# idthanm/mpg

Hardware: AMD Instinct MI355X
Metric: env-steps/sec + grad-steps/sec, PathTrackingEnv MPG n=25 batch=4096 (higher is better)
Workload: dtype f32-via-split-f16; 1 GPU; PathTrackingEnv, MPG-v2 learner, n=25, M=1, 4096 vectorised envs + replay batch 4096 per GPU; step = worker.sample(4096 env-steps) + add_batch + replay + compute_gradient + (all-reduce) + apply_gradients; global_batch=4096, parallelism=dp1, grad_allreduce_floats=205334, native_step_driver=True, always_exchange=False, overlap_exchange=False, rows_per_gpu=4096

## Files before the change

### mpg_amd/csrc/fused_kernels.hip

```cpp
#include "mlp_wgrad.h"

namespace mlp {

namespace {

template <bool PK>
__device__ __forceinline__ void load_w2(const float* pack, const float* W2, bool bwd, const Lane& L, float (&w)[128]) {
    if constexpr (PK) load_w2_packed(pack, L, w);
    else if (bwd) load_w2_bwd(W2, L, w);
    else load_w2_fwd(W2, L, w);
}

#define MPG_UNPAREN(...) __VA_ARGS__
#define MPG_LOAD2(SMALL, IMAGE) do { MPG_UNPAREN SMALL; MPG_UNPAREN IMAGE; } while (0)


constexpr int SMEM_FLOATS = 2 * A_IMG + GROUP * XS + NWAVE * GROUP * MAXOUT + GROUP * MAXOUT + NWAVE * GROUP * XS + 4 * GROUP;
struct Smem {
    float *sA, *sA1, *sX, *sPart, *sD3, *sPartX, *sQ;
    __device__ explicit Smem(float* base) {
        sA = base;
        sA1 = sA + A_IMG;
        sX = sA1 + A_IMG;
        sPart = sX + GROUP * XS;
        sD3 = sPart + NWAVE * GROUP * MAXOUT;
        sPartX = sD3 + GROUP * MAXOUT;
        sQ = sPartX + NWAVE * GROUP * XS;
    }
};

struct TargetArgs {
    const float *pol, *q1, *q2;
    const float *pk_pol, *pk_q1, *pk_q2;
    int rows;
    const float *obs2, *rew, *smooth_eps;
    float scale[8];
    int out_tanh;
    float out_scale, sigma, clipc, rshift, rscale, gamma;
    float* y;
    int draw, n_storage;
    int d_capacity, d_fresh_start, d_fresh_count;
    uint32_t dk0, dk1, dc1, dc2;
    const float *r_obs, *r_act, *r_rew, *r_obs2;
    const uint8_t* r_done;
    int* o_idx;
    float *o_obs, *o_act, *o_rew, *o_obs2, *o_done;
    int* status;
    float* qpart;
    unsigned long long* dbg;
};

template <int OBS, int ACT, bool PK, int G2>
__global__ void __launch_bounds__(NTHREAD, 2) k_target_fused(const TargetArgs a) {
    constexpr int QIN = OBS + ACT;
    __shared__ __attribute__((aligned(16))) float smem[SMEM_FLOATS];
    __shared__ __attribute__((aligned(16))) float sXg[G2][GROUP * XS];
    __shared__ float sQg[G2][2 * GROUP];
    const Smem m(smem);
    const Lane L;
    const int tid = threadIdx.x;
    const long g0 = (long)blockIdx.x * G2;
    const int half = a.qpart ? (int)blockIdx.y : -1;
    __shared__ float sRew[G2 * GROUP];
    MPG_TL_DECL
    MPG_TL(0);
    float o1[OBS], o2[OBS], ac[ACT], rw = 0.f;
    uint8_t dn = 0;
    long sr = 0;
    bool saw_nan = false;
#pragma unroll
    for (int i = 0; i < OBS; ++i) o1[i] = o2[i] = 0.f;
#pragma unroll
    for (int k = 0; k < ACT; ++k) ac[k] = 0.f;
    const bool drawn = a.draw && tid < G2 * GROUP && g0 * GROUP + tid < a.rows;
    bool gather = drawn;
    if (drawn) {
        const long gr = g0 * GROUP + tid;
        const Philox4 p = philox4x32_10((uint32_t)(gr >> 2), a.dc1, a.dc2, 0x1d5u, a.dk0, a.dk1);
        sr = (long)(((uint64_t)philox_word(p, (int)(gr & 3)) * (uint64_t)a.n_storage) >> 32);
        if (a.draw == 2) {
            int off = (int)sr - a.d_fresh_start;
            if (off < 0) off += a.d_capacity;
            gather = off < a.d_fresh_count;
        }
        if (gather) {
#pragma unroll
            for (int i = 0; i < OBS; ++i) { o1[i] = a.r_obs[sr * OBS + i]; o2[i] = a.r_obs2[sr * OBS + i]; }
#pragma unroll
            for (int k = 0; k < ACT; ++k) ac[k] = a.r_act[sr * ACT + k];
            rw = a.r_rew[sr];
            dn = a.r_done[sr];
        } else {
#pragma unroll
            for (int i = 0; i < OBS; ++i) o2[i] = a.o_obs2[gr * OBS + i];
            rw = a.o_rew[gr];
        }
    }
    float w2[128], h1[2][4], h2[2][4];
    float zmax = 0.f;
    const Net pnet = make_net(a.pol, OBS, 2 * ACT);
    float pb3 = 0.f, qb3[2] = {0.f, 0.f}, sm_eps = 0.f;
    if (tid < G2 * GROUP * ACT) {
        pb3 = pnet.b3[tid % ACT];
        const long gr0 = (g0 + tid / (GROUP * ACT)) * GROUP + (tid / ACT) % GROUP;
        if (a.smooth_eps && gr0 < a.rows) sm_eps = a.smooth_eps[gr0 * ACT + tid % ACT];
    }
    if (tid < G2 * GROUP) {
        qb3[0] = make_net(a.q1, OBS + ACT, 1).b3[0];
        if (a.q2) qb3[1] = make_net(a.q2, OBS + ACT, 1).b3[0];
    }
    SmallRegs<OBS, ACT> pr;
    MPG_TL(1);
    MPG_LOAD2((load_small<OBS, ACT>(pnet, L, pr)), (load_w2<PK>(a.pk_pol, pnet.W2, false, L, w2)));
    MPG_TL(2);
    if (a.draw) {
        if (tid < G2 * GROUP) {
            if (gather && half <= 0) {
                const long gr = g0 * GROUP + tid;
                if (a.o_idx) a.o_idx[gr] = (int)sr;
#pragma unroll
                for (int i = 0; i < OBS; ++i) { a.o_obs[gr * OBS + i] = o1[i]; a.o_obs2[gr * OBS + i] = o2[i]; }
#pragma unroll
                for (int k = 0; k < ACT; ++k) a.o_act[gr * ACT + k] = ac[k];
                a.o_rew[gr] = rw;
                if (a.o_done) a.o_done[gr] = (float)dn;
            }
            sRew[tid] = rw;
            saw_nan |= rw != rw;
#pragma unroll
            for (int i = 0; i < XS; ++i) sXg[tid / GROUP][(tid % GROUP) * XS + i] = i < OBS ? o2[i < OBS ? i : 0] * a.scale[i] : 0.f;
#pragma unroll
            for (int i = 0; i < OBS; ++i) saw_nan |= o2[i] != o2[i];
        }
    } else if (tid < G2 * GROUP * XS) {
        const int g2 = tid / (GROUP * XS), e = tid % (GROUP * XS), row = e / XS, i = e % XS;
        const long gr = (g0 + g2) * GROUP + row;
        const float xin = (gr < a.rows && i < OBS) ? a.obs2[gr * OBS + i] * a.scale[i] : 0.f;
        sXg[g2][e] = xin;
        saw_nan |= xin != xin;
        if (i == 0) {
            const float rin = gr < a.rows ? a.rew[gr] : 0.f;
            sRew[g2 * GROUP + row] = rin;
            saw_nan |= rin != rin;
        }
    }
    MPG_TL(3);
    lds_barrier();
    MPG_TL(4);
    float h1b[2][4], h2b[2][4];
    if constexpr (G2 == 2) {
        forward_group2<OBS, ACT>(sXg[0], sXg[1], m.sA, m.sA1, m.sPart, m.sPartX, L, w2, pr, h1, h2, h1b, h2b, &zmax);
    } else {
        forward_group<OBS, ACT>(sXg[0], m.sA, m.sPart, L, w2, pr, h1, h2, nullptr, 0, nullptr, &zmax);
    }
    if (tid < G2 * GROUP * ACT) {
        const int g2 = tid / (GROUP * ACT), row = (tid / ACT) % GROUP, k = tid % ACT;
        const long gr = (g0 + g2) * GROUP + row;
        const float z = out_preact(g2 == 0 ? m.sPart : m.sPartX, pb3, row, k);
        float act = a.out_tanh ? a.out_scale * tanhf(z) : z;
        if (a.smooth_eps && gr < a.rows) act += fminf(fmaxf(a.sigma * sm_eps, -a.clipc), a.clipc);
        sXg[g2][row * XS + OBS + k] = act;
    }
    MPG_TL(5);
    lds_barrier();
    MPG_TL(6);
#pragma unroll
    for (int qi = 0; qi < 2; ++qi) {
        const float* qp = qi == 0 ? a.q1 : a.q2;
        if (!qp) break;
        if (half >= 0 && qi != half) continue;
        const Net net = make_net(qp, QIN, 1);
        SmallRegs<QIN, 1> r;
        MPG_LOAD2((load_small<QIN, 1>(net, L, r)), (load_w2<PK>(qi == 0 ? a.pk_q1 : a.pk_q2, net.W2, false, L, w2)));
        MPG_TL(10 + 6 * qi);
        if constexpr (G2 == 2) {
            forward_group2<QIN, 1>(sXg[0], sXg[1], m.sA, m.sA1, m.sPart, m.sPartX, L, w2, r, h1, h2, h1b, h2b, &zmax);
        } else {
            forward_group<QIN, 1>(sXg[0], m.sA, m.sPart, L, w2, r, h1, h2, nullptr, 0, nullptr, &zmax);
        }
        if (tid < G2 * GROUP) {
            const int g2 = tid / GROUP, row = tid % GROUP;
            sQg[g2][qi * GROUP + row] = out_preact(g2 == 0 ? m.sPart : m.sPartX, qb3[qi], row, 0);
        }
        MPG_TL(11 + 6 * qi);
        lds_barrier();
        MPG_TL(12 + 6 * qi);
    }
    MPG_TL(22);
    if (tid < G2 * GROUP) {
        const int g2 = tid / GROUP, row = tid % GROUP;
        const long gr = (g0 + g2) * GROUP + row;
        if (gr < a.rows) {
            const float pz = row_poison(sXg[g2] + row * XS, OBS);
            if (half >= 0) a.qpart[(long)half * a.rows + gr] = sQg[g2][half * GROUP + row] + pz;
            else {
                const float q = a.q2 ? fminf(sQg[g2][row], sQg[g2][GROUP + row]) : sQg[g2][row];
                a.y[gr] = (sRew[tid] + a.rshift) * a.rscale + a.gamma * q + pz;
            }
        }
    }
    report_activation_range(a.status, zmax);
    report_nan(a.status, saw_nan);
    MPG_TL(23);
    MPG_TL_DUMP(a.dbg);
}

struct QlossArgs {
    const float* q[2];
    const float *pkf[2], *pkb[2];
    int rows;
    XSpec x;
    const float* y;
    float inv_b;
    CriticStash st[2];
    float* loss_part;
    float* td;
    int* status;
    const float* qpart;
    const float* rew;
    float rshift, rscale, gamma;
    float* y_out;
};

template <int QIN, bool PK>
__global__ void __launch_bounds__(NTHREAD, 2) k_qloss_fused(const QlossArgs a) {
    __shared__ __attribute__((aligned(16))) float smem[SMEM_FLOATS];
    const Smem m(smem);
    const Lane L;
    const int tid = threadIdx.x;
    const long g = blockIdx.x;
    const int qi = blockIdx.y;
    const long ngroups = gridDim.x;
    const Net net = make_net(a.q[qi], QIN, 1);
    const CriticStash st = a.st[qi];
    load_x_group<QIN>(a.x, a.rows, g, m.sX);
    lds_barrier();
    float w2[128], h1[2][4], h2[2][4], dz1[2][4], dz2[2][4];
    float zmax = 0.f;
    SmallRegs<QIN, 1> r;
    MPG_LOAD2((load_small<QIN, 1>(net, L, r)), (load_w2<PK>(a.pkf[qi], net.W2, false, L, w2)));
    forward_group<QIN, 1>(m.sX, m.sA, m.sPart, L, w2, r, h1, h2, nullptr, 0, nullptr, &zmax);
    report_activation_range(a.status, zmax);
    stash_store(st.h1, g, L, h1);
    stash_store(st.h2, g, L, h2);
    if (tid < GROUP) {
        const long gr = g * GROUP + tid;
        float e = 0.f;
        if (gr < a.rows) {
            e = out_preact(m.sPart, net.b3[0], tid, 0) - a.y[gr] + row_poison(m.sX + tid * XS, QIN);
            st.dz3[gr] = e * a.inv_b;
            if (a.td && qi == 0) a.td[gr] = e;
        }
        m.sD3[d3_index(tid, 0)] = e * a.inv_b;
        m.sQ[tid] = e * e;
        report_nan(a.status, e != e);
    }
// ... 227 lines not shown
    }
    if (slices && tid >= 64 && tid < 66) {
        const int sl = tid - 64;
        float s1 = 0.f, s2 = 0.f;
        for (int i = 0; i < GROUP; ++i) { const float v = sQ2[sl * GROUP + i]; s1 += v; s2 += v * v; }
        q.ret_part[(sl * ngroups + g) * 2] = s1;
        q.ret_part[(sl * ngroups + g) * 2 + 1] = s2;
    }
    backward_group<QIN, 1, false>(m.sD3, m.sA, m.sA1, m.sPartX, L, w2, r, h1[0], h2[0], dz1, dz2);
    stash_store(st.dz1, g, L, dz1);
    stash_store(st.dz2, g, L, dz2);
    MPG_TL(6);
    if (slices) {
#pragma unroll
        for (int sl = 0; sl < 2; ++sl) {
            backward_group<QIN, 1, true>(sD32 + sl * GROUP * MAXOUT, m.sA, m.sA1, m.sPartX, L, w2, r, h1[1 + sl], h2[1 + sl], dz1, dz2);
            if (tid < GROUP * QIN) {
                const int row = tid / QIN, i = tid % QIN;
                const long gr = (sl * ngroups + g) * GROUP + row;
                q.gxq[gr * QIN + i] = dx_reduce(m.sPartX, row, i);
            }
        }
    }
    MPG_TL(7);
#ifdef MPG_TIMELINE
    __syncthreads();
    if (ca.dbg && blockIdx.x == 7 && threadIdx.x < NWAVE * MPG_TL_MARKS)
        ca.dbg[blockIdx.y * NWAVE * MPG_TL_MARKS + threadIdx.x] = s_tl[threadIdx.x / MPG_TL_MARKS][threadIdx.x % MPG_TL_MARKS];
#endif
}

template <int QIN, bool PK>
__global__ void __launch_bounds__(NTHREAD, 2) k_critic_fused4(const CriticArgs ca) {
    constexpr int G4 = 4;
    __shared__ __attribute__((aligned(16))) float smem[SMEM_FLOATS];
    __shared__ __attribute__((aligned(16))) float sX4[G4 * GROUP * XS];
    __shared__ __attribute__((aligned(16))) float sD34[G4 * GROUP * MAXOUT];
    __shared__ float sQ4[G4 * GROUP];
    __shared__ __attribute__((aligned(16))) float sA2[A_IMG];
    __shared__ __attribute__((aligned(16))) float sPartX2[NWAVE * GROUP * XS];
    __shared__ __attribute__((aligned(16))) float sHold[8 * NTHREAD * 4];
    const QlossArgs& a = ca.ql;
    const QsliceArgs& q = ca.qs;
    const Smem m(smem);
    const Lane L;
    const int tid = threadIdx.x;
    const long ngroups = a.rows / GROUP;
    const long nq1 = 3 * ngroups / G4;
    const bool q2wg = (long)blockIdx.x >= nq1;
    const int qi = q2wg ? 1 : 0;
    const long u0 = (q2wg ? (long)blockIdx.x - nq1 : (long)blockIdx.x) * G4;
    const int kind = q2wg ? 0 : (int)(u0 / ngroups);
    const long g0 = u0 - (long)kind * ngroups;
    const bool slices = kind > 0;
    const int sl = kind > 0 ? kind - 1 : 0;
    const Net net = make_net(a.q[qi], QIN, 1);
    const CriticStash st = a.st[qi];
    float xv = 0.f;
    {
        const int u4 = tid / (GROUP * XS), e = tid % (GROUP * XS), row = e / XS, i = e % XS;
        const long gr = (g0 + u4) * GROUP + row;
        if (i < QIN) {
            if (slices) xv = q.xq[((long)sl * a.rows + gr) * QIN + i];
            else xv = i < a.x.d0 ? a.x.x0[gr * a.x.ld0 + i] * a.x.scale[i] : a.x.x1[gr * a.x.ld1 + (i - a.x.d0)];
        }
    }
    float t_y = 0.f, t_rew = 0.f, t_q1 = 0.f, t_q2 = 0.f, gk_in = 0.f;
    const float b3v = net.b3[0];
    if (tid < G4 * GROUP) {
        const long gr = (g0 + tid / GROUP) * GROUP + tid % GROUP;
        if (slices) gk_in = q.gk[(long)sl * a.rows + gr];
        else if (a.qpart) { t_rew = a.rew[gr]; t_q1 = a.qpart[gr]; t_q2 = a.qpart[(long)a.rows + gr]; }
        else t_y = a.y[gr];
    }
    float w2[128], h1[2][2][4], h2[2][2][4], dz1[2][4], dz2[2][4];
    float zmax = 0.f;
    SmallRegs<QIN, 1> r;
    MPG_LOAD2((load_small<QIN, 1>(net, L, r)), (load_w2<PK>(a.pkf[qi], net.W2, false, L, w2)));
    sX4[tid] = xv;
    if (slices) report_nan(a.status, xv != xv);
    lds_barrier();
#pragma unroll
    for (int p = 0; p < 2; ++p) {
        forward_group2<QIN, 1>(sX4 + (2 * p) * GROUP * XS, sX4 + (2 * p + 1) * GROUP * XS, m.sA, m.sA1, m.sPart, m.sPartX, L, w2, r,
                               h1[0], h2[0], h1[1], h2[1], &zmax);
        if (!slices) {
#pragma unroll
            for (int e = 0; e < 2; ++e) {
                stash_store(st.h1, g0 + 2 * p + e, L, h1[e]);
                stash_store(st.h2, g0 + 2 * p + e, L, h2[e]);
            }
        }
        if (p == 0) {
            f32x4* hold = reinterpret_cast<f32x4*>(sHold) + tid;
#pragma unroll
            for (int e = 0; e < 2; ++e)
#pragma unroll
                for (int t = 0; t < 2; ++t) {
                    hold[((e * 2 + 0) * 2 + t) * NTHREAD] = f32x4{h1[e][t][0], h1[e][t][1], h1[e][t][2], h1[e][t][3]};
                    hold[((e * 2 + 1) * 2 + t) * NTHREAD] = f32x4{h2[e][t][0], h2[e][t][1], h2[e][t][2], h2[e][t][3]};
                }
        }
        if (tid < G4 * GROUP && (tid >> 5) == p) {
            const int u4 = tid / GROUP, row = tid % GROUP;
            const long gr = (g0 + u4) * GROUP + row;
            const float qv = out_preact((u4 & 1) ? m.sPartX : m.sPart, b3v, row, 0);
            if (slices) {
                sQ4[tid] = gk_in + q.gpow[sl] * qv;
                sD34[u4 * GROUP * MAXOUT + d3_index(row, 0)] = q.coef[sl];
            } else {
                float yv = t_y;
                if (a.qpart) {
                    yv = (t_rew + a.rshift) * a.rscale + a.gamma * fminf(t_q1, t_q2);
                    if (qi == 0) a.y_out[gr] = yv;
                }
                const float e = qv - yv + row_poison(sX4 + tid * XS, QIN);
                st.dz3[gr] = e * a.inv_b;
                if (a.td && qi == 0) a.td[gr] = e;
                sD34[u4 * GROUP * MAXOUT + d3_index(row, 0)] = e * a.inv_b;
                sQ4[tid] = e * e;
                report_nan(a.status, e != e);
            }
        }
    }
    report_activation_range(a.status, zmax);
    load_w2<PK>(a.pkb[qi], net.W2, true, L, w2);
    lds_barrier();
    if (tid >= 64 && tid < 64 + G4) {
        const int u4 = tid - 64;
        float s1 = 0.f, s2 = 0.f;
        for (int i = 0; i < GROUP; ++i) { const float v = sQ4[u4 * GROUP + i]; s1 += v; s2 += v * v; }
        if (slices) {
            q.ret_part[((long)sl * ngroups + g0 + u4) * 2] = s1;
            q.ret_part[((long)sl * ngroups + g0 + u4) * 2 + 1] = s2;
        } else {
            a.loss_part[qi * ngroups + g0 + u4] = 0.5f * a.inv_b * s1;
        }
    }
    float dz1b[2][4], dz2b[2][4];
#pragma unroll
    for (int pass = 0; pass < 2; ++pass) {
        const int p = 1 - pass, ua = 2 * p, ub = 2 * p + 1;
        if (pass == 1) {
            const f32x4* hold = reinterpret_cast<const f32x4*>(sHold) + tid;
#pragma unroll
            for (int e = 0; e < 2; ++e)
#pragma unroll
                for (int t = 0; t < 2; ++t) {
                    const f32x4 x1 = hold[((e * 2 + 0) * 2 + t) * NTHREAD], x2 = hold[((e * 2 + 1) * 2 + t) * NTHREAD];
#pragma unroll
                    for (int j = 0; j < 4; ++j) { h1[e][t][j] = x1[j]; h2[e][t][j] = x2[j]; }
                }
        }
        if (slices) {
            backward_group2<QIN, 1, true>(sD34 + ua * GROUP * MAXOUT, sD34 + ub * GROUP * MAXOUT, m.sA, sA2, m.sA1, m.sPartX, sPartX2, L, w2, r,
                                          h1[0], h2[0], h1[1], h2[1], dz1, dz2, dz1b, dz2b);
            if (tid < 2 * GROUP * QIN) {
                const int e = tid / (GROUP * QIN), rem = tid % (GROUP * QIN), row = rem / QIN, i = rem % QIN;
                const long gr = ((long)sl * ngroups + g0 + ua + e) * GROUP + row;
                q.gxq[gr * QIN + i] = dx_reduce(e ? sPartX2 : m.sPartX, row, i);
            }
            if (pass == 0) lds_barrier();
        } else {
            backward_group2<QIN, 1, false>(sD34 + ua * GROUP * MAXOUT, sD34 + ub * GROUP * MAXOUT, m.sA, sA2, m.sA1, m.sPartX, sPartX2, L, w2, r,
                                           h1[0], h2[0], h1[1], h2[1], dz1, dz2, dz1b, dz2b);
            stash_store(st.dz1, g0 + ua, L, dz1);
            stash_store(st.dz2, g0 + ua, L, dz2);
            stash_store(st.dz1, g0 + ub, L, dz1b);
            stash_store(st.dz2, g0 + ub, L, dz2b);
        }
    }
}

struct WgradMulti {
    int n_jobs;
    WgradArgs a[3];
    int type[3];
    int chunk_off[4];
    int chunk0;
    unsigned long long* dbg;
};

#ifndef MPG_WGM_WAVES
#define MPG_WGM_WAVES 4
#endif
template <int IA, int OA, int IB, int OB>
__global__ void __launch_bounds__(NTHREAD, MPG_WGM_WAVES) k_wgrad_multi(const WgradMulti m) {
    constexpr int NQA = wgrad_nq<IA, OA>(), NQB = wgrad_nq<IB, OB>();
    __shared__ __attribute__((aligned(16))) float sRed[NWAVE * (NQA > NQB ? NQA : NQB) * 64];
    int gchunk, sl;
#if defined(MPG_SPLIT)
    const int nch = gridDim.x / 12;
    const int role = (int)blockIdx.x < 4 * nch ? 1 : 2;
    if (role == 1) wgrad_map4(blockIdx.x, nch, gchunk, sl);
    else wgrad_map((int)blockIdx.x - 4 * nch, nch, gchunk, sl);
#else
    const int role = 0;
    wgrad_map(blockIdx.x, gridDim.x >> 3, gchunk, sl);
#endif
    gchunk += m.chunk0;
    int j = 0;
    while (j + 1 < m.n_jobs && gchunk >= m.chunk_off[j + 1]) ++j;
    const int chunk = gchunk - m.chunk_off[j];
    MPG_TL_DECL
    MPG_TL(0);
#if defined(MPG_SPLIT)
    if (role == 1) {
        if (m.type[j] == 0) wgrad_body<IA, OA, 1, 4>(m.a[j], sl, chunk, sRed);
        else wgrad_body<IB, OB, 1, 4>(m.a[j], sl, chunk, sRed);
// ... 338 lines not shown
```

### mpg_amd/csrc/mlp_core.h

```cpp
#pragma once
#include "mpg_common.h"

namespace mlp {

constexpr int H = 256;
constexpr int NTHREAD = 512;
constexpr int NWAVE = 8;
constexpr int GROUP = 16;
constexpr int A_IMG = 4608;
constexpr int LDA = 280;
constexpr int KS = 68;
constexpr int XS = 8;
template <int IN>
__host__ __device__ constexpr int xs_of() { return IN <= 8 ? 8 : (IN <= 16 ? 16 : 24); }
template <int IN>
__host__ __device__ constexpr int l1_steps() { return IN <= 8 ? 2 : (IN <= 16 ? 4 : 6); }
template <int OU>
__host__ __device__ constexpr int out_stride() { return OU <= 2 ? 2 : 4; }
constexpr int MAXOUT = out_stride<2>();

typedef float f32x4 __attribute__((ext_vector_type(4)));

#ifndef MPG_F32_MFMA
#define MPG_SPLIT 1
#endif
typedef _Float16 f16x8 __attribute__((ext_vector_type(8)));
typedef _Float16 f16x2 __attribute__((ext_vector_type(2)));
constexpr int ROW_H = 72, PLANE_H = GROUP * ROW_H, IMG_H = 4 * PLANE_H;
__device__ __forceinline__ int h_index(int row, int k) { return ((k >> 3) & 3) * PLANE_H + row * ROW_H + 8 * (k >> 5) + (k & 7); }
typedef short s16x4 __attribute__((__vector_size__(4 * sizeof(short))));
typedef unsigned u32x2 __attribute__((ext_vector_type(2)));
constexpr float W_SCALE = 64.f;
constexpr float A_SCALE = 16.f;
constexpr float H_LIMIT = 65504.f / A_SCALE;
constexpr float P_LIMIT = 65504.f / W_SCALE;
__device__ __forceinline__ float max8(const float (&a)[4], const float (&b)[4], float m) {
    m = __builtin_fmaxf(__builtin_fmaxf(a[0], a[1]), m);
    m = __builtin_fmaxf(__builtin_fmaxf(a[2], a[3]), m);
    m = __builtin_fmaxf(__builtin_fmaxf(b[0], b[1]), m);
    m = __builtin_fmaxf(__builtin_fmaxf(b[2], b[3]), m);
    return m;
}
__device__ __forceinline__ void report_activation_range(int* status, float zmax) {
    if (status && !(zmax < H_LIMIT)) atomicOr(status, MPG_STATUS_ACTIVATION_RANGE);
}

__device__ __forceinline__ void split_pack2(float w0, float w1, float& hi_word, float& lo_word) {
    const f16x2 hi = {(_Float16)w0, (_Float16)w1};
    const f16x2 lo = {(_Float16)(w0 - (float)hi[0]), (_Float16)(w1 - (float)hi[1])};
    hi_word = __builtin_bit_cast(float, hi);
    lo_word = __builtin_bit_cast(float, lo);
}

__device__ __forceinline__ float w_scaled(float w) { return fminf(fmaxf(w * W_SCALE, -65504.f), 65504.f); }

struct Net {
    const float *W1, *b1, *W2, *b2, *W3, *b3;
    int in_dim, out_dim;
};

__host__ __device__ inline int net_size(int in_dim, int out_dim) {
    return in_dim * H + H + H * H + H + H * out_dim + out_dim;
}

__host__ __device__ inline Net make_net(const float* p, int in_dim, int out_dim) {
    Net n;
    n.in_dim = in_dim;
    n.out_dim = out_dim;
    n.W1 = p;
    n.b1 = n.W1 + in_dim * H;
    n.W2 = n.b1 + H;
    n.b2 = n.W2 + H * H;
    n.W3 = n.b2 + H;
    n.b3 = n.W3 + H * out_dim;
    return n;
}

struct Lane {
    int lane, wave, c, rg;
    __device__ Lane() {
        lane = threadIdx.x & 63;
        wave = threadIdx.x >> 6;
        c = lane & 15;
        rg = lane >> 4;
    }
    __device__ int col(int t) const { return 32 * wave + 16 * t + c; }
    __device__ int row(int j) const { return 4 * rg + j; }
};

__device__ __forceinline__ void prefer_young_waves() {
    if (threadIdx.x >= 256) __builtin_amdgcn_s_setprio(1);
}

__device__ __forceinline__ void lds_barrier() { asm volatile("s_waitcnt lgkmcnt(0)\n\ts_barrier" ::: "memory"); }

#ifdef MPG_TIMELINE
#define MPG_TL_MARKS 24
__shared__ unsigned long long s_tl[8][MPG_TL_MARKS];
#define MPG_TL_DECL
#define MPG_TL(k) do { __builtin_amdgcn_sched_barrier(0); if ((threadIdx.x & 63) == 0) s_tl[threadIdx.x >> 6][k] = __builtin_amdgcn_s_memtime(); __builtin_amdgcn_sched_barrier(0); } while (0)
#define MPG_TL_DUMP(dbg) do { __syncthreads(); if (dbg && (blockIdx.x == 0 || blockIdx.x == 100) && threadIdx.x < NWAVE * MPG_TL_MARKS) \
    dbg[(blockIdx.x ? 1 : 0) * NWAVE * MPG_TL_MARKS + threadIdx.x] = s_tl[threadIdx.x / MPG_TL_MARKS][threadIdx.x % MPG_TL_MARKS]; } while (0)
#else
#define MPG_TL_DECL
#define MPG_TL(k)
#define MPG_TL_DUMP(dbg)
#endif
// ... 112 lines not shown
#pragma unroll
        for (int t = 0; t < 2; ++t)
#pragma unroll
            for (int r = 0; r < 4; ++r) {
                const int k0 = 32 * kb + 8 * L.rg + 2 * r;
                split_pack2(w_scaled(W2[L.col(t) * H + k0]), w_scaled(W2[L.col(t) * H + k0 + 1]),
                            w[4 * ((kb * 2 + t) * 2) + r], w[4 * ((kb * 2 + t) * 2 + 1) + r]);
                if (r == 3) __builtin_amdgcn_sched_barrier(0);
            }
}
__host__ __device__ constexpr int img_slot(int wave, int v) {
    return wave * 32 + v;
}
__host__ __device__ inline void img_unslot(int slot, int& wave, int& v) {
    wave = slot >> 5; v = slot & 31;
}
__device__ __forceinline__ void load_w2_packed(const float* __restrict__ pack, const Lane& L, float (&w)[128]) {
    const f32x4* p = reinterpret_cast<const f32x4*>(pack) + L.lane;
#pragma unroll
    for (int v = 0; v < 32; ++v) {
        const f32x4 q = p[img_slot(L.wave, v) * 64];
#pragma unroll
        for (int e = 0; e < 4; ++e) w[4 * v + e] = q[e];
    }
}
#else
__device__ __forceinline__ void load_w2_fwd(const float* __restrict__ W2, const Lane& L, float (&w)[128]) {
#pragma unroll
    for (int q = 0; q < 64; ++q)
#pragma unroll
        for (int t = 0; t < 2; ++t) w[2 * q + t] = W2[(4 * q + L.rg) * H + L.col(t)];
}
__device__ __forceinline__ void load_w2_bwd(const float* __restrict__ W2, const Lane& L, float (&w)[128]) {
#pragma unroll
    for (int q = 0; q < 64; ++q)
#pragma unroll
        for (int t = 0; t < 2; ++t) w[2 * q + t] = W2[L.col(t) * H + 4 * q + L.rg];
}

__device__ __forceinline__ void load_w2_packed(const float* __restrict__ pack, const Lane& L, float (&w)[128]) {
    const f32x4* p = reinterpret_cast<const f32x4*>(pack) + (L.wave * 32) * 64 + L.lane;
#pragma unroll
    for (int q4 = 0; q4 < 16; ++q4)
#pragma unroll
        for (int t = 0; t < 2; ++t) {
            const f32x4 v = p[(q4 * 2 + t) * 64];
#pragma unroll
            for (int e = 0; e < 4; ++e) w[2 * (4 * q4 + e) + t] = v[e];
        }
}
#endif

const float* weight_cache_lookup(const mpg_cfg_t* cfg, const float* W2, int dir);
const float* wcache_lookup(const mpg_wcache_t* wc, const float* W2, int dir);
int wcache_w2_offset(const mpg_wcache_t* wc, int k);

#ifdef MPG_SPLIT
__device__ __forceinline__ void mfma_16x256x32(const float* sA, const Lane& L, const float (&w)[128], f32x4& acc0,
                                               f32x4& acc1) {
    const _Float16* bh = reinterpret_cast<const _Float16*>(sA) + L.rg * PLANE_H + L.c * ROW_H;
    const _Float16* bl = bh + IMG_H;
    constexpr int NKB = 8;
    auto frag = [&](int v) {
        return __builtin_bit_cast(f16x8, f32x4{w[4 * v], w[4 * v + 1], w[4 * v + 2], w[4 * v + 3]});
    };
    f32x4 m0 = {0.f, 0.f, 0.f, 0.f}, m1 = m0;
#pragma unroll
    for (int kb = 0; kb < NKB; ++kb) {
        const f16x8 ah = *reinterpret_cast<const f16x8*>(bh + 8 * kb), al = *reinterpret_cast<const f16x8*>(bl + 8 * kb);
        const int v0 = (kb * 2 + 0) * 2, v1 = (kb * 2 + 1) * 2;
        m0 = __builtin_amdgcn_mfma_f32_16x16x32_f16(ah, frag(v0), m0, 0, 0, 0);
        m1 = __builtin_amdgcn_mfma_f32_16x16x32_f16(ah, frag(v1), m1, 0, 0, 0);
        m0 = __builtin_amdgcn_mfma_f32_16x16x32_f16(ah, frag(v0 + 1), m0, 0, 0, 0);
        m1 = __builtin_amdgcn_mfma_f32_16x16x32_f16(ah, frag(v1 + 1), m1, 0, 0, 0);
        m0 = __builtin_amdgcn_mfma_f32_16x16x32_f16(al, frag(v0), m0, 0, 0, 0);
        m1 = __builtin_amdgcn_mfma_f32_16x16x32_f16(al, frag(v1), m1, 0, 0, 0);
    }
#pragma unroll
    for (int j = 0; j < 4; ++j) {
        acc0[j] = fmaf(m0[j], 1.f / (W_SCALE * A_SCALE), acc0[j]);
        acc1[j] = fmaf(m1[j], 1.f / (W_SCALE * A_SCALE), acc1[j]);
    }
}
#else
__device__ __forceinline__ void mfma_16x256x32(const float* sA, const Lane& L, const float (&w)[128], f32x4& acc0,
                                               f32x4& acc1) {
    const float* base = sA + L.c * LDA + L.rg * KS;
    constexpr int NQ4 = 16;
    f32x4 a = *reinterpret_cast<const f32x4*>(base);
#pragma unroll
    for (int q4 = 0; q4 < NQ4; ++q4) {
        f32x4 nxt = a;
        if (q4 + 1 < NQ4) nxt = *reinterpret_cast<const f32x4*>(base + 4 * (q4 + 1));
#pragma unroll
        for (int i = 0; i < 4; ++i) {
            acc0 = __builtin_amdgcn_mfma_f32_16x16x4f32(a[i], w[2 * (4 * q4 + i)], acc0, 0, 0, 0);
            acc1 = __builtin_amdgcn_mfma_f32_16x16x4f32(a[i], w[2 * (4 * q4 + i) + 1], acc1, 0, 0, 0);
        }
        a = nxt;
    }
}
#endif

template <int IN, int OU>
struct SmallRegs {
    float w1p[l1_steps<IN>()][2];
    float w1t[8];
    float w1t2[IN > 16 ? 8 : 1];
    float b1[2], b2[2];
    float w3[2][OU];
};

template <int IN, int OU>
__device__ __forceinline__ void load_small(const Net& n, const Lane& L, SmallRegs<IN, OU>& r) {
    static_assert(IN <= 24, "layer-1 MFMA covers K <= 24");
#pragma unroll
    for (int q = 0; q < 8; ++q) r.w1t[q] = L.c < n.in_dim ? n.W1[L.c * H + 32 * L.wave + 4 * q + L.rg] : 0.f;
    if constexpr (IN > 16) {
#pragma unroll
        for (int q = 0; q < 8; ++q) r.w1t2[q] = 16 + L.c < n.in_dim ? n.W1[(16 + L.c) * H + 32 * L.wave + 4 * q + L.rg] : 0.f;
    }
#pragma unroll
    for (int t = 0; t < 2; ++t) {
        const int col = L.col(t);
#pragma unroll
        for (int q = 0; q < l1_steps<IN>(); ++q) r.w1p[q][t] = (4 * q + L.rg) < n.in_dim ? n.W1[(4 * q + L.rg) * H + col] : 0.f;
        r.b1[t] = n.b1[col];
        r.b2[t] = n.b2[col];
#pragma unroll
        for (int o = 0; o < OU; ++o) r.w3[t][o] = n.W3[col * n.out_dim + o];
    }
}

template <int IN, int OU>
__device__ __forceinline__ void dx_partials(const SmallRegs<IN, OU>& r, const Lane& L, const f32x4& a0, const f32x4& a1, float* sPartX) {
    f32x4 dx = {0.f, 0.f, 0.f, 0.f};
#pragma unroll
    for (int q = 0; q < 4; ++q) dx = __builtin_amdgcn_mfma_f32_16x16x4f32(a0[q], r.w1t[q], dx, 0, 0, 0);
#pragma unroll
    for (int q = 0; q < 4; ++q) dx = __builtin_amdgcn_mfma_f32_16x16x4f32(a1[q], r.w1t[4 + q], dx, 0, 0, 0);
    if (L.c < xs_of<IN>()) {
#pragma unroll
        for (int j = 0; j < 4; ++j) sPartX[(L.wave * GROUP + L.row(j)) * xs_of<IN>() + L.c] = dx[j];
    }
    if constexpr (IN > 16) {
        f32x4 dx2 = {0.f, 0.f, 0.f, 0.f};
#pragma unroll
        for (int q = 0; q < 4; ++q) dx2 = __builtin_amdgcn_mfma_f32_16x16x4f32(a0[q], r.w1t2[q], dx2, 0, 0, 0);
#pragma unroll
        for (int q = 0; q < 4; ++q) dx2 = __builtin_amdgcn_mfma_f32_16x16x4f32(a1[q], r.w1t2[4 + q], dx2, 0, 0, 0);
        if (16 + L.c < xs_of<IN>()) {
#pragma unroll
            for (int j = 0; j < 4; ++j) sPartX[(L.wave * GROUP + L.row(j)) * xs_of<IN>() + 16 + L.c] = dx2[j];
        }
    }
}

enum class StashStore { plain, write_through };
enum class StashLoad { plain, nontemporal };
template <StashStore P = StashStore::plain>
__device__ __forceinline__ void stash_store(float* __restrict__ base, long group, const Lane& L, const float (&v)[2][4]) {
    f32x4* p = reinterpret_cast<f32x4*>(base) + (group * 16 + 2 * L.wave) * 64 + L.lane;
    const f32x4 a = {v[0][0], v[0][1], v[0][2], v[0][3]}, b = {v[1][0], v[1][1], v[1][2], v[1][3]};
    if constexpr (P == StashStore::write_through) {
        asm volatile("global_store_dwordx4 %0, %1, off sc1\n\tglobal_store_dwordx4 %0, %2, off offset:1024 sc1\n\ts_nop 1"
                     :: "v"(p), "v"(a), "v"(b) : "memory");
    } else {
        p[0] = a;
        p[64] = b;
    }
}
template <StashLoad P = StashLoad::plain>
__device__ __forceinline__ void stash_load(const float* __restrict__ base, long group, const Lane& L, float (&v)[2][4]) {
    const f32x4* p = reinterpret_cast<const f32x4*>(base) + (group * 16 + 2 * L.wave) * 64 + L.lane;
    f32x4 a, b;
    if constexpr (P == StashLoad::nontemporal) {
        a = __builtin_nontemporal_load(p);
        b = __builtin_nontemporal_load(p + 64);
    } else {
        a = p[0];
        b = p[64];
    }
#pragma unroll
    for (int j = 0; j < 4; ++j) {
        v[0][j] = a[j];
        v[1][j] = b[j];
    }
}

template <int IN, int OU, bool FINAL_BARRIER = true, StashStore ST = StashStore::plain>
__device__ __forceinline__ void forward_group(const float* sX, float* sA, float* sPart, const Lane& L,
                                              const float (&w2)[128], const SmallRegs<IN, OU>& r,
                                              float (&h1)[2][4], float (&h2)[2][4], float* h1_stash = nullptr,
                                              long stash_group = 0, const float* xa_regs = nullptr, float* zmax = nullptr) {
    {
        f32x4 z0 = {r.b1[0], r.b1[0], r.b1[0], r.b1[0]}, z1 = {r.b1[1], r.b1[1], r.b1[1], r.b1[1]};
#pragma unroll
        for (int q = 0; q < l1_steps<IN>(); ++q) {
            const float xa = xa_regs ? xa_regs[q] : sX[L.c * xs_of<IN>() + 4 * q + L.rg];
            z0 = __builtin_amdgcn_mfma_f32_16x16x4f32(xa, r.w1p[q][0], z0, 0, 0, 0);
            z1 = __builtin_amdgcn_mfma_f32_16x16x4f32(xa, r.w1p[q][1], z1, 0, 0, 0);
        }
        elu8(z0, z1, h1);
        if (zmax) *zmax = max8(h1[0], h1[1], *zmax);
    }
    store_c_to_a(sA, L, h1);
    if (h1_stash) stash_store<ST>(h1_stash, stash_group, L, h1);
    MPG_STAMP_AT(1);
    lds_barrier();
    MPG_STAMP_AT(2);
    f32x4 acc0 = {r.b2[0], r.b2[0], r.b2[0], r.b2[0]};
    f32x4 acc1 = {r.b2[1], r.b2[1], r.b2[1], r.b2[1]};
    mfma_16x256x32(sA, L, w2, acc0, acc1);
    MPG_STAMP_AT(3);
    elu8(acc0, acc1, h2);
    {
        float p[OU][4];
#pragma unroll
        for (int o = 0; o < OU; ++o)
#pragma unroll
            for (int j = 0; j < 4; ++j) p[o][j] = fmaf(h2[1][j], r.w3[1][o], h2[0][j] * r.w3[0][o]);
#define MPG_DPP_STAGE(MODS)                                     \
        _Pragma("unroll") for (int o = 0; o < OU; ++o)           \
        _Pragma("unroll") for (int j = 0; j < 4; ++j)            \
            asm volatile("v_add_f32_dpp %0, %1, %1 " MODS " row_mask:0xf bank_mask:0xf" : "=v"(p[o][j]) : "v"(p[o][j]));
        static_assert(OU == 1 || OU == 2 || OU == 4, "the wait below names every p[o][j]");
        if constexpr (OU == 4)
            asm volatile("s_nop 1" : "+v"(p[0][0]), "+v"(p[0][1]), "+v"(p[0][2]), "+v"(p[0][3]), "+v"(p[1][0]), "+v"(p[1][1]),
                         "+v"(p[1][2]), "+v"(p[1][3]), "+v"(p[2][0]), "+v"(p[2][1]), "+v"(p[2][2]), "+v"(p[2][3]), "+v"(p[OU - 1][0]),
                         "+v"(p[OU - 1][1]), "+v"(p[OU - 1][2]), "+v"(p[OU - 1][3]));
        else if constexpr (OU == 2)
            asm volatile("s_nop 1" : "+v"(p[0][0]), "+v"(p[0][1]), "+v"(p[0][2]), "+v"(p[0][3]), "+v"(p[OU - 1][0]),
                         "+v"(p[OU - 1][1]), "+v"(p[OU - 1][2]), "+v"(p[OU - 1][3]));
        else
            asm volatile("s_nop 1" : "+v"(p[0][0]), "+v"(p[0][1]), "+v"(p[0][2]), "+v"(p[0][3]));
        MPG_DPP_STAGE("quad_perm:[1,0,3,2]") MPG_DPP_STAGE("quad_perm:[2,3,0,1]")
        MPG_DPP_STAGE("row_half_mirror") MPG_DPP_STAGE("row_mirror")
#undef MPG_DPP_STAGE
        if (L.c == 0) {
#pragma unroll
            for (int o = 0; o < OU; ++o)
#pragma unroll
                for (int j = 0; j < 4; ++j) sPart[(L.wave * GROUP + L.row(j)) * out_stride<OU>() + o] = p[o][j];
        }
    }
    MPG_STAMP_AT(4);
    if (FINAL_BARRIER) {
        lds_barrier();
        MPG_STAMP_AT(5);
    }
}

template <int IN, int OU>
__device__ __forceinline__ void forward_group2(const float* sXa, const float* sXb, float* sAa, float* sAb, float* sPartA,
                                               float* sPartB, const Lane& L, const float (&w2)[128], const SmallRegs<IN, OU>& r,
                                               float (&h1a)[2][4], float (&h2a)[2][4], float (&h1b)[2][4], float (&h2b)[2][4],
                                               float* zmax = nullptr) {
    auto layer1 = [&](const float* sX, float* sA, float (&h1)[2][4]) {
        f32x4 z0 = {r.b1[0], r.b1[0], r.b1[0], r.b1[0]}, z1 = {r.b1[1], r.b1[1], r.b1[1], r.b1[1]};
#pragma unroll
        for (int q = 0; q < l1_steps<IN>(); ++q) {
            const float xa = sX[L.c * xs_of<IN>() + 4 * q + L.rg];
            z0 = __builtin_amdgcn_mfma_f32_16x16x4f32(xa, r.w1p[q][0], z0, 0, 0, 0);
            z1 = __builtin_amdgcn_mfma_f32_16x16x4f32(xa, r.w1p[q][1], z1, 0, 0, 0);
        }
        elu8(z0, z1, h1);
        if (zmax) *zmax = max8(h1[0], h1[1], *zmax);
        store_c_to_a(sA, L, h1);
    };
    auto output = [&](float* sPart, const float (&h2)[2][4]) {
        float p[OU][4];
#pragma unroll
        for (int o = 0; o < OU; ++o)
#pragma unroll
            for (int j = 0; j < 4; ++j) p[o][j] = fmaf(h2[1][j], r.w3[1][o], h2[0][j] * r.w3[0][o]);
#define MPG_DPP_STAGE(MODS)                                     \
        _Pragma("unroll") for (int o = 0; o < OU; ++o)           \
        _Pragma("unroll") for (int j = 0; j < 4; ++j)            \
            asm volatile("v_add_f32_dpp %0, %1, %1 " MODS " row_mask:0xf bank_mask:0xf" : "=v"(p[o][j]) : "v"(p[o][j]));
        static_assert(OU == 1 || OU == 2 || OU == 4, "the wait below names every p[o][j]");
        if constexpr (OU == 4)
            asm volatile("s_nop 1" : "+v"(p[0][0]), "+v"(p[0][1]), "+v"(p[0][2]), "+v"(p[0][3]), "+v"(p[1][0]), "+v"(p[1][1]),
                         "+v"(p[1][2]), "+v"(p[1][3]), "+v"(p[2][0]), "+v"(p[2][1]), "+v"(p[2][2]), "+v"(p[2][3]), "+v"(p[OU - 1][0]),
                         "+v"(p[OU - 1][1]), "+v"(p[OU - 1][2]), "+v"(p[OU - 1][3]));
        else if constexpr (OU == 2)
            asm volatile("s_nop 1" : "+v"(p[0][0]), "+v"(p[0][1]), "+v"(p[0][2]), "+v"(p[0][3]), "+v"(p[OU - 1][0]),
                         "+v"(p[OU - 1][1]), "+v"(p[OU - 1][2]), "+v"(p[OU - 1][3]));
        else
            asm volatile("s_nop 1" : "+v"(p[0][0]), "+v"(p[0][1]), "+v"(p[0][2]), "+v"(p[0][3]));
        MPG_DPP_STAGE("quad_perm:[1,0,3,2]") MPG_DPP_STAGE("quad_perm:[2,3,0,1]")
        MPG_DPP_STAGE("row_half_mirror") MPG_DPP_STAGE("row_mirror")
#undef MPG_DPP_STAGE
        if (L.c == 0) {
#pragma unroll
            for (int o = 0; o < OU; ++o)
#pragma unroll
                for (int j = 0; j < 4; ++j) sPart[(L.wave * GROUP + L.row(j)) * out_stride<OU>() + o] = p[o][j];
        }
    };
    layer1(sXa, sAa, h1a);
    layer1(sXb, sAb, h1b);
    lds_barrier();
    f32x4 a0 = {r.b2[0], r.b2[0], r.b2[0], r.b2[0]}, a1 = {r.b2[1], r.b2[1], r.b2[1], r.b2[1]};
    f32x4 b0 = a0, b1 = a1;
    mfma_16x256x32(sAa, L, w2, a0, a1);
    mfma_16x256x32(sAb, L, w2, b0, b1);
    elu8(a0, a1, h2a);
    elu8(b0, b1, h2b);
    output(sPartA, h2a);
    output(sPartB, h2b);
    lds_barrier();
}

template <int OS = MAXOUT>
__device__ __forceinline__ float out_preact(const float* sPart, float bias, int row, int o) {
    float z = bias;
#pragma unroll
    for (int w = 0; w < NWAVE; ++w) z += sPart[(w * GROUP + row) * OS + o];
    return z;
}
__device__ __forceinline__ float out_preact_tree(const float* sPart, float bias, int row, int o) {
    float p[NWAVE];
#pragma unroll
    for (int w = 0; w < NWAVE; ++w) p[w] = sPart[(w * GROUP + row) * MAXOUT + o];
    return (((p[0] + p[1]) + (p[2] + p[3])) + ((p[4] + p[5]) + (p[6] + p[7]))) + bias;
}

__device__ __forceinline__ int d3_index(int row, int o) { return o * GROUP + row; }

template <int OU>
__device__ __forceinline__ void row_exponents(const float* sD3, const Lane& L, int (&e)[4]) {
    f32x4 m = {0.f, 0.f, 0.f, 0.f};
#pragma unroll
    for (int o = 0; o < OU; ++o) {
        const f32x4 d = *reinterpret_cast<const f32x4*>(sD3 + o * GROUP + 4 * L.rg);
#pragma unroll
        for (int j = 0; j < 4; ++j) m[j] = fmaxf(m[j], fabsf(d[j]));
    }
#pragma unroll
    for (int j = 0; j < 4; ++j) e[j] = __builtin_amdgcn_frexp_expf(m[j]);
}

template <int IN, int OU>
__device__ __forceinline__ void backward_dz2(const float* sD3, float* sA, const Lane& L, const SmallRegs<IN, OU>& r,
                                             const float (&h2)[2][4], float (&dz2)[2][4]) {
    f32x4 d3v[OU];
#pragma unroll
    for (int o = 0; o < OU; ++o) d3v[o] = *reinterpret_cast<const f32x4*>(sD3 + d3_index(4 * L.rg, o));
#pragma unroll
    for (int j = 0; j < 4; ++j) {
#pragma unroll
        for (int t = 0; t < 2; ++t) {
            float dh = 0.f;
#pragma unroll
            for (int o = 0; o < OU; ++o) dh = fmaf(d3v[o][j], r.w3[t][o], dh);
            dz2[t][j] = dh * elu_grad_from_out(h2[t][j]);
        }
    }
#ifdef MPG_SPLIT
    {
        int e[4];
        row_exponents<OU>(sD3, L, e);
        float sc[2][4];
#pragma unroll
        for (int t = 0; t < 2; ++t)
#pragma unroll
            for (int j = 0; j < 4; ++j) sc[t][j] = ldexpf(dz2[t][j], -e[j]);
        store_c_to_a(sA, L, sc);
    }
#else
    store_c_to_a(sA, L, dz2);
#endif
    MPG_STAMP_AT(1);
    lds_barrier();
    MPG_STAMP_AT(2);
}

template <int IN, int OU, bool WANT_DX, bool FINAL_BARRIER = true>
__device__ __forceinline__ void backward_rest(const float* sD3, float* sA, float* sA1, float* sPartX, const Lane& L,
                                              const float (&w2t)[128], const SmallRegs<IN, OU>& r, const float (&h1)[2][4],
                                              float (&dz1)[2][4]) {
    f32x4 acc0 = {0.f, 0.f, 0.f, 0.f}, acc1 = {0.f, 0.f, 0.f, 0.f};
    mfma_16x256x32(sA, L, w2t, acc0, acc1);
    MPG_STAMP_AT(3);
#ifdef MPG_SPLIT
    int e[4];
    row_exponents<OU>(sD3, L, e);
#endif
#pragma unroll
// ... 142 lines not shown
```

Before: 18.89 million env-steps/s.

## Prefetch next layer-2 weight image during final MFMA sweep of current network

Adds an MFMA loop variant that, once each k-block's weight fragments have been consumed, overwrites those register slots with the next network's packed W2 image loaded from global memory. Scheduling barriers pin MFMA issue between the loads. The policy forward prefetches the first Q network's weights and small params, and the critic forward prefetches the backward weight image, so the separate loads before the next stage are skipped. The aim is to hide global weight-load latency behind matrix math, at the cost of extra live registers and a const_cast that mutates the weight array. It applies only to the packed split-f16 path.

```diff
diff --git a/mpg_amd/csrc/fused_kernels.hip b/mpg_amd/csrc/fused_kernels.hip
--- a/mpg_amd/csrc/fused_kernels.hip
+++ b/mpg_amd/csrc/fused_kernels.hip
@@ -10,6 +10,9 @@
     else if (bwd) load_w2_bwd(W2, L, w);
     else load_w2_fwd(W2, L, w);
 }
+
+template <bool PK>
+constexpr bool NXT = PK && HAS_NEXT_IMG;
 
 #define MPG_UNPAREN(...) __VA_ARGS__
 #define MPG_LOAD2(SMALL, IMAGE) do { MPG_UNPAREN SMALL; MPG_UNPAREN IMAGE; } while (0)
@@ -112,6 +115,10 @@
     SmallRegs<OBS, ACT> pr;
     MPG_TL(1);
     MPG_LOAD2((load_small<OBS, ACT>(pnet, L, pr)), (load_w2<PK>(a.pk_pol, pnet.W2, false, L, w2)));
+    const int q_first = half == 1 ? 1 : 0;
+    SmallRegs<QIN, 1> r;
+    if constexpr (NXT<PK>) load_small<QIN, 1>(make_net(q_first ? a.q2 : a.q1, QIN, 1), L, r);
+    const float* const pk_first = q_first ? a.pk_q2 : a.pk_q1;
     MPG_TL(2);
     if (a.draw) {
         if (tid < G2 * GROUP) {
@@ -149,9 +156,9 @@
     MPG_TL(4);
     float h1b[2][4], h2b[2][4];
     if constexpr (G2 == 2) {
-        forward_group2<OBS, ACT>(sXg[0], sXg[1], m.sA, m.sA1, m.sPart, m.sPartX, L, w2, pr, h1, h2, h1b, h2b, &zmax);
+        forward_group2<OBS, ACT, NXT<PK>>(sXg[0], sXg[1], m.sA, m.sA1, m.sPart, m.sPartX, L, w2, pr, h1, h2, h1b, h2b, &zmax, pk_first);
     } else {
-        forward_group<OBS, ACT>(sXg[0], m.sA, m.sPart, L, w2, pr, h1, h2, nullptr, 0, nullptr, &zmax);
+        forward_group<OBS, ACT, true, StashStore::plain, NXT<PK>>(sXg[0], m.sA, m.sPart, L, w2, pr, h1, h2, nullptr, 0, nullptr, &zmax, pk_first);
     }
     if (tid < G2 * GROUP * ACT) {
         const int g2 = tid / (GROUP * ACT), row = (tid / ACT) % GROUP, k = tid % ACT;
@@ -170,8 +177,8 @@
         if (!qp) break;
         if (half >= 0 && qi != half) continue;
         const Net net = make_net(qp, QIN, 1);
-        SmallRegs<QIN, 1> r;
-        MPG_LOAD2((load_small<QIN, 1>(net, L, r)), (load_w2<PK>(qi == 0 ? a.pk_q1 : a.pk_q2, net.W2, false, L, w2)));
+        if (!(NXT<PK> && qi == q_first))
+            MPG_LOAD2((load_small<QIN, 1>(net, L, r)), (load_w2<PK>(qi == 0 ? a.pk_q1 : a.pk_q2, net.W2, false, L, w2)));
         MPG_TL(10 + 6 * qi);
         if constexpr (G2 == 2) {
             forward_group2<QIN, 1>(sXg[0], sXg[1], m.sA, m.sA1, m.sPart, m.sPartX, L, w2, r, h1, h2, h1b, h2b, &zmax);
@@ -565,8 +572,12 @@
     lds_barrier();
 #pragma unroll
     for (int p = 0; p < 2; ++p) {
-        forward_group2<QIN, 1>(sX4 + (2 * p) * GROUP * XS, sX4 + (2 * p + 1) * GROUP * XS, m.sA, m.sA1, m.sPart, m.sPartX, L, w2, r,
-                               h1[0], h2[0], h1[1], h2[1], &zmax);
+        if (NXT<PK> && p == 1)
+            forward_group2<QIN, 1, NXT<PK>>(sX4 + 2 * GROUP * XS, sX4 + 3 * GROUP * XS, m.sA, m.sA1, m.sPart, m.sPartX, L, w2, r,
+                                            h1[0], h2[0], h1[1], h2[1], &zmax, a.pkb[qi]);
+        else
+            forward_group2<QIN, 1>(sX4 + (2 * p) * GROUP * XS, sX4 + (2 * p + 1) * GROUP * XS, m.sA, m.sA1, m.sPart, m.sPartX, L, w2, r,
+                                   h1[0], h2[0], h1[1], h2[1], &zmax);
         if (!slices) {
 #pragma unroll
             for (int e = 0; e < 2; ++e) {
@@ -607,7 +618,7 @@
         }
     }
     report_activation_range(a.status, zmax);
-    load_w2<PK>(a.pkb[qi], net.W2, true, L, w2);
+    if constexpr (!NXT<PK>) load_w2<PK>(a.pkb[qi], net.W2, true, L, w2);
     lds_barrier();
     if (tid >= 64 && tid < 64 + G4) {
         const int u4 = tid - 64;
diff --git a/mpg_amd/csrc/mlp_core.h b/mpg_amd/csrc/mlp_core.h
--- a/mpg_amd/csrc/mlp_core.h
+++ b/mpg_amd/csrc/mlp_core.h
@@ -23,6 +23,11 @@
 
 #ifndef MPG_F32_MFMA
 #define MPG_SPLIT 1
+#endif
+#ifdef MPG_SPLIT
+constexpr bool HAS_NEXT_IMG = true;
+#else
+constexpr bool HAS_NEXT_IMG = false;
 #endif
 typedef _Float16 f16x8 __attribute__((ext_vector_type(8)));
 typedef _Float16 f16x2 __attribute__((ext_vector_type(2)));
@@ -301,6 +306,52 @@
         acc1[j] = fmaf(m1[j], 1.f / (W_SCALE * A_SCALE), acc1[j]);
     }
 }
+__device__ __forceinline__ void mfma_16x256x32_then_load(const float* sA, const Lane& L, float (&w)[128], f32x4& acc0, f32x4& acc1,
+                                                         const float* __restrict__ next_pack) {
+    const _Float16* bh = reinterpret_cast<const _Float16*>(sA) + L.rg * PLANE_H + L.c * ROW_H;
+    const _Float16* bl = bh + IMG_H;
+    const char* np = reinterpret_cast<const char*>(next_pack) + (size_t)__builtin_amdgcn_readfirstlane(L.wave) * (32 * 1024);
+    const unsigned lane_off = (unsigned)L.lane * 16u;
+    constexpr int NKB = 8;
+    auto frag = [&](int v) {
+        return __builtin_bit_cast(f16x8, f32x4{w[4 * v], w[4 * v + 1], w[4 * v + 2], w[4 * v + 3]});
+    };
+    f32x4 m0 = {0.f, 0.f, 0.f, 0.f}, m1 = m0;
+#define MPG_PIN_MFMA __builtin_amdgcn_sched_barrier(0x7F6)
+#define MPG_PIN_MFMA_VMEM __builtin_amdgcn_sched_barrier(0x786)
+#pragma unroll
+    for (int kb = 0; kb < NKB; ++kb) {
+        const f16x8 ah = *reinterpret_cast<const f16x8*>(bh + 8 * kb), al = *reinterpret_cast<const f16x8*>(bl + 8 * kb);
+        const int v0 = (kb * 2 + 0) * 2, v1 = (kb * 2 + 1) * 2;
+        m0 = __builtin_amdgcn_mfma_f32_16x16x32_f16(ah, frag(v0), m0, 0, 0, 0);
+        MPG_PIN_MFMA;
+        m1 = __builtin_amdgcn_mfma_f32_16x16x32_f16(ah, frag(v1), m1, 0, 0, 0);
+        MPG_PIN_MFMA;
+        m0 = __builtin_amdgcn_mfma_f32_16x16x32_f16(ah, frag(v0 + 1), m0, 0, 0, 0);
+        MPG_PIN_MFMA;
+        m1 = __builtin_amdgcn_mfma_f32_16x16x32_f16(ah, frag(v1 + 1), m1, 0, 0, 0);
+        MPG_PIN_MFMA;
+        m0 = __builtin_amdgcn_mfma_f32_16x16x32_f16(al, frag(v0), m0, 0, 0, 0);
+        MPG_PIN_MFMA;
+        m1 = __builtin_amdgcn_mfma_f32_16x16x32_f16(al, frag(v1), m1, 0, 0, 0);
+        MPG_PIN_MFMA_VMEM;
+        const unsigned off = lane_off + kb * 4096;
+#pragma unroll
+        for (int v = 0; v < 4; ++v) {
+            const f32x4 q = *reinterpret_cast<const f32x4*>(np + ((size_t)off + v * 1024));
+#pragma unroll
+            for (int e = 0; e < 4; ++e) w[4 * (4 * kb + v) + e] = q[e];
+        }
+        MPG_PIN_MFMA_VMEM;
+    }
+#undef MPG_PIN_MFMA
+#undef MPG_PIN_MFMA_VMEM
+#pragma unroll
+    for (int j = 0; j < 4; ++j) {
+        acc0[j] = fmaf(m0[j], 1.f / (W_SCALE * A_SCALE), acc0[j]);
+        acc1[j] = fmaf(m1[j], 1.f / (W_SCALE * A_SCALE), acc1[j]);
+    }
+}
 #else
 __device__ __forceinline__ void mfma_16x256x32(const float* sA, const Lane& L, const float (&w)[128], f32x4& acc0,
                                                f32x4& acc1) {
@@ -407,11 +458,12 @@
     }
 }
 
-template <int IN, int OU, bool FINAL_BARRIER = true, StashStore ST = StashStore::plain>
+template <int IN, int OU, bool FINAL_BARRIER = true, StashStore ST = StashStore::plain, bool NEXT_IMG = false>
 __device__ __forceinline__ void forward_group(const float* sX, float* sA, float* sPart, const Lane& L,
                                               const float (&w2)[128], const SmallRegs<IN, OU>& r,
                                               float (&h1)[2][4], float (&h2)[2][4], float* h1_stash = nullptr,
-                                              long stash_group = 0, const float* xa_regs = nullptr, float* zmax = nullptr) {
+                                              long stash_group = 0, const float* xa_regs = nullptr, float* zmax = nullptr,
+                                              const float* next_pack = nullptr) {
     {
         f32x4 z0 = {r.b1[0], r.b1[0], r.b1[0], r.b1[0]}, z1 = {r.b1[1], r.b1[1], r.b1[1], r.b1[1]};
 #pragma unroll
@@ -430,7 +482,13 @@
     MPG_STAMP_AT(2);
     f32x4 acc0 = {r.b2[0], r.b2[0], r.b2[0], r.b2[0]};
     f32x4 acc1 = {r.b2[1], r.b2[1], r.b2[1], r.b2[1]};
-    mfma_16x256x32(sA, L, w2, acc0, acc1);
+#ifdef MPG_SPLIT
+    if constexpr (NEXT_IMG) mfma_16x256x32_then_load(sA, L, const_cast<float (&)[128]>(w2), acc0, acc1, next_pack);
+    else
+#else
+    static_assert(!NEXT_IMG, "the trailing image request exists in the split engine only");
+#endif
+        mfma_16x256x32(sA, L, w2, acc0, acc1);
     MPG_STAMP_AT(3);
     elu8(acc0, acc1, h2);
     {
@@ -470,11 +528,11 @@
     }
 }
 
-template <int IN, int OU>
+template <int IN, int OU, bool NEXT_IMG = false>
 __device__ __forceinline__ void forward_group2(const float* sXa, const float* sXb, float* sAa, float* sAb, float* sPartA,
                                                float* sPartB, const Lane& L, const float (&w2)[128], const SmallRegs<IN, OU>& r,
                                                float (&h1a)[2][4], float (&h2a)[2][4], float (&h1b)[2][4], float (&h2b)[2][4],
-                                               float* zmax = nullptr) {
+                                               float* zmax = nullptr, const float* next_pack = nullptr) {
     auto layer1 = [&](const float* sX, float* sA, float (&h1)[2][4]) {
         f32x4 z0 = {r.b1[0], r.b1[0], r.b1[0], r.b1[0]}, z1 = {r.b1[1], r.b1[1], r.b1[1], r.b1[1]};
 #pragma unroll
@@ -523,7 +581,13 @@
     f32x4 a0 = {r.b2[0], r.b2[0], r.b2[0], r.b2[0]}, a1 = {r.b2[1], r.b2[1], r.b2[1], r.b2[1]};
     f32x4 b0 = a0, b1 = a1;
     mfma_16x256x32(sAa, L, w2, a0, a1);
-    mfma_16x256x32(sAb, L, w2, b0, b1);
+#ifdef MPG_SPLIT
+    if constexpr (NEXT_IMG) mfma_16x256x32_then_load(sAb, L, const_cast<float (&)[128]>(w2), b0, b1, next_pack);
+    else
+#else
+    static_assert(!NEXT_IMG, "the trailing image request exists in the split engine only");
+#endif
+        mfma_16x256x32(sAb, L, w2, b0, b1);
     elu8(a0, a1, h2a);
     elu8(b0, b1, h2b);
     output(sPartA, h2a);
```

Result: no change. 18.83 million env-steps/s (-0.3%).
